# EdinburghGenomics/well_duplicates

Hardware: AMD Instinct MI355X
Metric: target x neighbour seq-compares/sec (whole node) (higher is better)
Workload: dtype u8; 1 GPU; 1 lane(s) x 96 tiles (hiseq_x) x 2500 targets x 5 levels, 50 bp; one lane per GPU (BASELINE configs[1]); lanes_per_rank=1, resident_bytes_per_rank=21098102688, mode=eq, k=0, early_exit=True, clusters_per_tile=4309253, valid_targets_per_rank=168032, parallelism=tiles sharded, 1 rank(s)

## Files before the change

### well_duplicates_amd/csrc/scan_queue.inc

```
constexpr int kFinishAllMax = 64;
#ifndef WD_QCAP
#define WD_QCAP 128
#endif
#ifndef WD_Q_OCC_IL
#define WD_Q_OCC_IL 8
#endif
constexpr int kQCap = WD_QCAP;
#ifndef WD_Q_DEPTH
#define WD_Q_DEPTH 1
#endif
constexpr int kQDepth = WD_Q_DEPTH;
constexpr int kFinishInPlace = 40;
static_assert(kQCap >= kPass && kQCap >= kFinishAllMax,
              "after a drain one pass must fit the queue, and q_finish_all adds up its pieces in the idle queue buffer");

template <typename T>
__device__ inline T late_arg(int offset)
{
    static_assert(sizeof(T) == 4 || sizeof(T) == 8, "one or two dwords");
    const __attribute__((address_space(4))) char *kp =
        (const __attribute__((address_space(4))) char *)__builtin_amdgcn_kernarg_segment_ptr();
    T v;
    if constexpr (sizeof(T) == 8)
        asm volatile("s_load_dwordx2 %0, %1, %2\n\ts_waitcnt lgkmcnt(0)" : "=s"(v) : "s"(kp), "s"(offset) : "memory");
    else
        asm volatile("s_load_dword %0, %1, %2\n\ts_waitcnt lgkmcnt(0)" : "=s"(v) : "s"(kp), "s"(offset) : "memory");
    return v;
}
#define WD_LATE_ARG(field) late_arg<decltype(ScanArgs::field)>((int)offsetof(ScanArgs, field))

struct QEnv {
    const int32_t *s_centre;
    const int32_t *s_off;
    uint32_t *s_d;
    const uint32_t *s_tid;
    gbytes base0;
    const uint8_t *const *ptab;
    int64_t stride;
    int levels, L, k, tile, t_first;
};

template <bool STRIDED, int WS = 1>
__device__ inline gbytes q_plane(const QEnv &v, int j)
{
    if (WS == 4)
        return v.base0 + (int64_t)(j >> 2) * v.stride + (j & 3);
    return STRIDED ? v.base0 + (int64_t)j * v.stride : as_global(v.ptab[j]);
}

__device__ inline void q_record_dup(const QEnv &v, int tl, int e, int dist)
{
    const int32_t *o = v.s_off + tl * (v.levels + 1);
    const int rel0 = o[0];
    int lev = 0;
    for (int l = 1; l < v.levels; l++)
        lev += (e >= o[l] - rel0) ? 1 : 0;
    atomicAdd(&v.s_d[tl * v.levels + lev], 1u);
    if (WD_LATE_ARG(log_hits)) {
        gptr<const ScanRare> rp = as_gptr(WD_LATE_ARG(rare));
        gptr<const int32_t> perm = as_gptr(WD_LATE_ARG(perm));
        wd_hit *const hits = rp->hits;
        const long long hit_cap = rp->hit_cap;
// ... 324 lines not shown
                alive = lev2_alive(st);
                if (last && alive)
                    q_record_dup(v, tl, (int)(ent.y & 0xFFFu), lev2_dist(st));
            }
            if (!last) {
                const uint64_t m = __ballot(alive);
                if (alive) {
                    const int pos = n2 + __builtin_amdgcn_mbcnt_hi((uint32_t)(m >> 32),
                                             __builtin_amdgcn_mbcnt_lo((uint32_t)m, 0u));
                    qb[pos] = make_uint2(idx, (ent.y & 0xFF000FFFu) | (st << 12));
                }
                n2 += __popcll(m);
            }
        }
        q_wave_sync();
        uint2 *t = qa; qa = qb; qb = t;
        n = last ? 0 : n2;
        j += nb;
        nb = WS == 4 ? NB : (nb < 4 ? nb * 2 : NB);
    }
    qn = 0;
}

constexpr int kLev2Closed = -1;
template <bool STRIDED, int B1, int LEVH = 0, int WS = 1>
__global__ __launch_bounds__(kBlock, LEVH > 0 ? 4 : (WS == 4 ? WD_Q_OCC_IL : 6)) void k_scan_q(ScanArgs a)
{
    static_assert(WS == 1 || (WS == 4 && STRIDED && ((B1 == 4 && LEVH == 0) || (B1 == 8 && (LEVH == 1 || LEVH == kLev2Closed)))),
                  "the interleaved layout is read a dword (4 cycles) at a time: one for equality / Hamming, "
                  "two for the first round of Levenshtein <= 2 / <= 3");
    using Entry = typename std::conditional<LEVH <= 0, uint2, uint4>::type;
    using LevS = LevState<(LEVH > 0 ? LEVH : 1)>;
    extern __shared__ uint32_t smem[];
    const int lane = threadIdx.x & (kWave - 1);
    const int wave = __builtin_amdgcn_readfirstlane(threadIdx.x >> 6);
    const int levels = a.levels;
    const int L = a.L;
    const int k = a.k;
    const int tpb = a.tpb;
    const int ncnt = 1 + 5 * levels;
    const int chunks = (a.T + tpb - 1) / tpb;
    const int nb = (int)gridDim.x, per_xcd = (nb + kXcds - 1) / kXcds;
    int vb = (int)(blockIdx.x % kXcds) * per_xcd + (int)(blockIdx.x / kXcds);
    if (nb % kXcds) {
        const int big = nb % kXcds, x = (int)(blockIdx.x % kXcds), small = nb / kXcds;
        vb = (x < big ? x * (small + 1) : big * (small + 1) + (x - big) * small) + (int)(blockIdx.x / kXcds);
    }
    const int tile = vb / chunks;
    const int chunk = vb - tile * chunks;
    const int t_first = chunk * tpb;
    const int n_t = min(tpb, a.T - t_first);

    uint32_t *s_cnt = smem;
    int32_t *s_centre = (int32_t *)(s_cnt + ncnt);
    int32_t *s_off = s_centre + tpb;
    uint32_t *s_d = (uint32_t *)(s_off + tpb * (levels + 1));
    uint32_t *s_valid = s_d + tpb * levels;
    uint32_t *s_items = s_valid + tpb;
    uint32_t *s_misc = s_items + kMaxPasses * tpb;
    const int q_base = (int)((((s_misc + 4) - smem) + 3) & ~3);
    Entry *q_a = (Entry *)(smem + q_base) + wave * 2 * kQCap;
    Entry *q_b = q_a + kQCap;

    gbytes filt = as_global(a.filter[tile]);
    const uint8_t *const *ptab = STRIDED ? nullptr : a.planes + (size_t)tile * L;
    gbytes base0 = STRIDED ? as_global(a.planes[tile]) : nullptr;
// ... 100 lines not shown
                for (int q = 0; q < NW; q++) {
                    w0[g][q] = w0[g - 1][q];
                    w1[g][q] = w1[g - 1][q];
                }
            }

            {
                it0 = s_items[wave + kWaves * min(s, n_my - 1)];
                const int tl = (int)(it0 >> 8);
                const int base = (int)(it0 & 0xFFu) * kPass;
                const int off0 = __builtin_amdgcn_readfirstlane(s_off[tl * (levels + 1)]);
                const int K = __builtin_amdgcn_readfirstlane(s_off[tl * (levels + 1) + levels]) - off0;
                const int e0 = base + lane, e1 = e0 + kWave;
                i0_0 = (uint32_t)a.nbr[off0 + min(e0, K - 1)];
                i1_0 = (uint32_t)a.nbr[off0 + min(e1, K - 1)];
            }
            if (lane == kWave - 1)
                i1_2 = (uint32_t)s_centre[it[SB] >> 8];
            if (WS == 4) {
#pragma unroll
                for (int g = 0; g < B1 / 4; g++) {
                    const int64_t go = (int64_t)min(g, max((L + 3) / 4 - 1, 0)) * stride;
                    w0_2[g] = *(const __attribute__((address_space(1))) uint32_t *)(base0 + go + (size_t)i0_2 * 4);
                    w1_2[g] = *(const __attribute__((address_space(1))) uint32_t *)(base0 + go + (size_t)i1_2 * 4);
                }
            } else if (L > 0) {
#pragma unroll
                for (int q = 0; q < B1; q++) {
                    w0_2[q] = ldb(pp[q], i0_2);
                    w1_2[q] = ldb(pp[q], i1_2);
                }
            }
            if (s >= AGE) {
                const int tl = (int)(it3 >> 8);
                const int base = (int)(it3 & 0xFFu) * kPass;
                const int off0 = __builtin_amdgcn_readfirstlane(s_off[tl * (levels + 1)]);
                const int K = __builtin_amdgcn_readfirstlane(s_off[tl * (levels + 1) + levels]) - off0;
                const int e0 = base + lane, e1 = e0 + kWave;
                const bool a0 = e0 < K, a1 = lane < kWave - 1 && e1 < K;
                if constexpr (LEVH == 0) {
                    int mm0 = 0, mm1 = 0;
                    if constexpr (WS == 4) {
                        static_assert(B1 == 4, "one dword is the first round");
                        const uint32_t cw = lev2_codes4((uint32_t)__builtin_amdgcn_readlane((int)w1_3[0], kWave - 1));
                        const uint32_t keep = L >= 4 ? (kLev2Nib & 0xFFFFu) : (((1u << (4 * L)) - 1u) & kLev2Nib);
                        const uint32_t y0 = lev2_codes4(w0_3[0]) ^ cw, y1 = lev2_codes4(w1_3[0]) ^ cw;
                        mm0 = __popc((y0 | (y0 >> 1) | (y0 >> 2)) & keep);
                        mm1 = __popc((y1 | (y1 >> 1) | (y1 >> 2)) & keep);
                    } else {
#pragma unroll
                        for (int q = 0; q < B1; q++) {
                            if (q < L) {
                                const uint32_t cc = code_of((uint32_t)__builtin_amdgcn_readlane((int)w1_3[q], kWave - 1));
                                mm0 += code_of(w0_3[q]) != cc ? 1 : 0;
                                mm1 += code_of(w1_3[q]) != cc ? 1 : 0;
                            }
                        }
                    }
                    const bool al0 = a0 && mm0 <= k, al1 = a1 && mm1 <= k;
                    const uint64_t m0 = __ballot(al0), m1 = __ballot(al1);
                    if (m0 | m1) {
                        if (B1 >= L) {
                            if (al0)
                                q_record_dup(env, tl, e0, mm0);
                            if (al1)
                                q_record_dup(env, tl, e1, mm1);
// ... 136 lines not shown
                        s1.finish(L, ch, cap, k);
                        if (a0 && s0.dup(k))
                            q_record_dup(env, tl, e0, s0.dist());
                        if (a1 && s1.dup(k))
                            q_record_dup(env, tl, e1, s1.dist());
                    } else {
                        const bool al0 = a0 && s0.alive(k, B1, ch, L, cap);
                        const bool al1 = a1 && s1.alive(k, B1, ch, L, cap);
                        const uint64_t m0 = __ballot(al0), m1 = __ballot(al1);
                        if (m0 | m1) {
                            const int n0 = __popcll(m0), n1 = __popcll(m1);
                            if (qn + n0 + n1 > kQCap)
                                q_drain_lev<STRIDED, (LEVH > 0 ? LEVH : 1), WS>(env, (uint4 *)q_a, (uint4 *)q_b, qn, B1, lane);
                            if (al0) {
                                const int pos = qn + __builtin_amdgcn_mbcnt_hi((uint32_t)(m0 >> 32),
                                                         __builtin_amdgcn_mbcnt_lo((uint32_t)m0, 0u));
                                const uint64_t pk = lev_pack(s0, ch);
                                ((uint4 *)q_a)[pos] = make_uint4(i0_3, ((uint32_t)tl << 24) | (uint32_t)e0,
                                                                 (uint32_t)pk, (uint32_t)(pk >> 32));
                            }
                            if (al1) {
                                const int pos = qn + n0 + __builtin_amdgcn_mbcnt_hi((uint32_t)(m1 >> 32),
                                                              __builtin_amdgcn_mbcnt_lo((uint32_t)m1, 0u));
                                const uint64_t pk = lev_pack(s1, ch);
                                ((uint4 *)q_a)[pos] = make_uint4(i1_3, ((uint32_t)tl << 24) | (uint32_t)e1,
                                                                 (uint32_t)pk, (uint32_t)(pk >> 32));
                            }
                            qn += n0 + n1;
                        }
                    }
                }
            }
        }
        if (qn > 0) {
            if constexpr (LEVH == 0)
                q_drain<STRIDED, 8, WS>(env, (uint2 *)q_a, (uint2 *)q_b, qn, B1, lane);
            else if constexpr (LEVH == kLev2Closed)
                q_drain_lev2<STRIDED, WS>(env, (uint2 *)q_a, (uint2 *)q_b, qn, B1, lane);
            else
                q_drain_lev<STRIDED, LEVH, WS>(env, (uint4 *)q_a, (uint4 *)q_b, qn, B1, lane);
        }
    }
    __syncthreads();

    uint32_t acc_wells = 0, acc_dups = 0, acc_hit = 0, acc_first = 0, acc_last = 0, acc_valid = 0;
    gptr<uint32_t> const out_pt = as_gptr(WD_LATE_ARG(out_per_target));
    gptr<const int32_t> const perm = out_pt ? as_gptr(WD_LATE_ARG(perm)) : nullptr;
    const size_t T_all = (size_t)WD_LATE_ARG(T);
    for (int tl = wave; tl < n_t; tl += kWaves) {
        const bool valid = __builtin_amdgcn_readfirstlane(s_valid[tl]) != 0;
        gptr<uint32_t> opt = out_pt ? out_pt + ((size_t)tile * T_all + (perm ? perm[t_first + tl] : t_first + tl)) * levels
                                    : nullptr;
        if (!valid) {
            if (opt && lane < levels)
                opt[lane] = WD_INVALID_TARGET;
            continue;
        }
        uint32_t my_d = 0, my_w = 0;
        if (lane < levels) {
            my_d = s_d[tl * levels + lane];
            my_w = (uint32_t)(s_off[tl * (levels + 1) + lane + 1] - s_off[tl * (levels + 1) + lane]);
        }
        const uint64_t hm = __ballot(lane < levels && my_d > 0);
        acc_valid += 1;
        acc_wells += my_w;
        acc_dups += my_d;
        acc_hit += my_d ? 1u : 0u;
        if (hm) {
            acc_first += (lane == __ffsll((long long)hm) - 1) ? 1u : 0u;
            acc_last += (lane == 63 - __clzll((long long)hm)) ? 1u : 0u;
        }
        if (opt && lane < levels)
            opt[lane] = my_d;
    }
    if (lane < levels) {
        if (acc_wells) atomicAdd(&s_cnt[1 + lane], acc_wells);
        if (acc_dups) atomicAdd(&s_cnt[1 + levels + lane], acc_dups);
        if (acc_hit) atomicAdd(&s_cnt[1 + 2 * levels + lane], acc_hit);
        if (acc_first) atomicAdd(&s_cnt[1 + 3 * levels + lane], acc_first);
        if (acc_last) atomicAdd(&s_cnt[1 + 4 * levels + lane], acc_last);
    }
    if (lane == 0 && acc_valid)
        atomicAdd(&s_cnt[0], acc_valid);
    __syncthreads();
    unsigned long long *const out_tile = WD_LATE_ARG(out_tile);
    for (int i = threadIdx.x; i < ncnt; i += kBlock) {
        const uint32_t v = s_cnt[i];
        if (v)
            g_atomic_add(&out_tile[(size_t)tile * ncnt + i], (unsigned long long)v);
    }
}
```

### well_duplicates_amd/csrc/wd_ctx.h

```cpp
#ifndef WD_CTX_H
#define WD_CTX_H
#include "wd_shared.h"

constexpr int kLaneTopMaxPasses = 8;

struct wd_ctx {
    int device = 0;
    hipStream_t own_stream = nullptr;
    hipStream_t stream = nullptr;
    std::string err;

    int early_exit = 1;
    int tpb = 64;
    int batch_first = 4;
    int batch_next = 4;
    int queue_kernel = 1;
    int queue_first = 0;
    int dense_kernel = -1;
    int dense_tile_chunk = 16;
    uint32_t *d_sig = nullptr;
    size_t sig_cap = 0;
    unsigned long long *d_partial = nullptr;
    size_t partial_cap = 0;
    uint32_t *d_mask = nullptr;
// ... 28 lines not shown
    int64_t P = 0;
    int32_t *d_centre = nullptr, *d_lvl_off = nullptr, *d_nbr = nullptr;
    int64_t idx_min = 0, idx_max = -1;
    int64_t k_max = 0;
    std::vector<long long> h_gbase;
    void *d_nbr_t = nullptr;
    bool nbr_t16 = false;
    int32_t *d_rel_t = nullptr;
    void *d_udelta = nullptr;
    uint8_t *d_guni = nullptr;
    int32_t *d_ginfo = nullptr;
    uint16_t *d_uoff = nullptr;
    int2 *d_useg = nullptr;
    int32_t *d_wdelta = nullptr;
    uint8_t *d_wlev = nullptr;
    uint32_t *d_wmask = nullptr;
    uint8_t *d_wfull = nullptr;
    int dense_sym = 1;
    bool dense_sym_on = false;
    int32_t centre0 = 0;
    int win_kpad = 0;
    int win_dwords = 0;
    long long n_uniform_groups = -1, n_window_groups = -1;
    int32_t *d_pblocks = nullptr;
    int n_pblocks = 0;
    uint32_t *d_tblflags = nullptr;
    long long *d_gbase = nullptr;
    bool has_targets = false;
    bool has_empty_level = false;

    std::vector<const uint8_t *> h_tbl;
    const uint8_t **d_tbl = nullptr;
    size_t d_tbl_cap = 0;
    uint32_t *d_status = nullptr;
    uint32_t *h_status = nullptr;
    ScanRare *d_rare = nullptr;
    ScanRare h_rare = {nullptr, nullptr, nullptr, 0};

    unsigned long long *d_out_tile = nullptr;
    size_t d_out_tile_cap = 0;
    uint32_t *d_out_pt = nullptr;
    size_t d_out_pt_cap = 0;
    uint8_t *d_stage = nullptr;
    size_t d_stage_cap = 0;

    wd_hit *d_hits = nullptr;
    unsigned long long *d_hit_count = nullptr;
    int64_t hit_cap = 0;
    uint8_t *d_gather = nullptr;
    size_t gather_cap = 0;
    size_t hit_alloc = 0;

    std::vector<std::pair<hipEvent_t, hipEvent_t>> events;
    std::vector<std::pair<hipEvent_t, hipEvent_t>> free_events;
    double prof_ms = 0.0;
    int64_t prof_launches = 0;

    void *comm = nullptr;

    struct IngestSlot {
        uint8_t *pinned = nullptr;
        size_t cap = 0;
        uint8_t *dev = nullptr;
        size_t dev_cap = 0;
        uint8_t *file = nullptr;
        size_t file_cap = 0;
// ... 135 lines not shown
```

### well_duplicates_amd/csrc/wd_shared.h

```cpp
#ifndef WD_SHARED_H
#define WD_SHARED_H
#include <hip/hip_runtime.h>

#include <dlfcn.h>
#include <zlib.h>
#include <stdint.h>
#include <stdio.h>
#include <stdlib.h>
#include <string.h>

#include <fcntl.h>
#include <emmintrin.h>
#include <sched.h>
#include <sys/stat.h>
#include <unistd.h>

#include <algorithm>
#include <atomic>
#include <chrono>
#include <condition_variable>
#include <functional>
#include <new>
#include <system_error>
#include <memory>
// ... 6 lines not shown

#include "welldup.h"

constexpr int kWave = 64;
constexpr int kBlock = 256;
constexpr int kWaves = kBlock / kWave;
constexpr int kMaxLevels = WD_MAX_LEVELS;
constexpr int kCounters = 1 + 5 * kMaxLevels;
constexpr uint32_t kStatusEmptyLevel = 1u;
constexpr int kXcds = 8;
constexpr int kMaxTpb = 64;
constexpr int kPass = 127;
constexpr int kMaxPasses = 4;

constexpr int lev_first(int H) { return H == 1 ? 7 : H == 2 ? 10 : H == 3 ? 13 : H == 4 ? 16 : H <= 6 ? 20 : 24; }

constexpr int kDenseChainVersion = 5;
constexpr int kSigCycles = 10;
constexpr int kRowGroups = 4;
constexpr int kDenseMaxK = 1 << 17;

struct ScanArgs {
    const uint8_t *const *planes;
    const uint8_t *const *filter;
    int64_t stride;
    const int32_t *centre;
    const int32_t *lvl_off;
    const int32_t *nbr;
    unsigned long long *out_tile;
    uint32_t *out_per_target;
    const struct ScanRare *rare;
    const int32_t *perm;
    int T, levels, L, k, tpb, early, check_empty, log_hits;
};

struct ScanRare {
    uint32_t *status;
    wd_hit *hits;
    unsigned long long *hit_count;
    long long hit_cap;
};

struct InfJob;
struct InfResult;

#endif
```

### well_duplicates_amd/csrc/welldup_core.hip

```cpp
#include "wd_ctx.h"

namespace {

#include "synth_kernels.inc"

struct Id128 { char b[WD_UNIQUE_ID_BYTES]; };
struct Rccl {
    void *handle = nullptr;
    int (*GetUniqueId)(void *) = nullptr;
    int (*CommInitRank)(void **, int, Id128, int) = nullptr;
    int (*AllReduce)(const void *, void *, size_t, int, int, void *, hipStream_t) = nullptr;
    int (*CommDestroy)(void *) = nullptr;
    const char *(*GetErrorString)(int) = nullptr;
};
Rccl g_rccl;

bool rccl_load(std::string &err)
{
    if (g_rccl.handle)
        return true;
    const char *names[] = {"librccl.so.1", "librccl.so", "/opt/rocm/lib/librccl.so.1"};
    void *h = nullptr;
    for (const char *n : names) {
        h = dlopen(n, RTLD_NOW | RTLD_GLOBAL);
// ... 148 lines not shown
void wd_destroy(wd_ctx *ctx)
{
    if (!ctx)
        return;
    (void)hipSetDevice(ctx->device);
    (void)hipStreamSynchronize(ctx->stream);
    if (ctx->fast_exit) {
        (void)hipDeviceSynchronize();
        if (ctx->comm && g_rccl.CommDestroy)
            g_rccl.CommDestroy(ctx->comm);
        delete ctx;
        return;
    }
    const bool lap_on = getenv("WD_INFLATE_STATS") != nullptr;
    auto lap_t = std::chrono::steady_clock::now();
    auto lap = [&](const char *what) {
        if (!lap_on)
            return;
        const auto now = std::chrono::steady_clock::now();
        fprintf(stderr, "[wd close] %-28s %6.1f ms\n", what, 1e3 * std::chrono::duration<double>(now - lap_t).count());
        lap_t = now;
    };
    drain_events(ctx);
    for (auto &ev : ctx->free_events) {
        (void)hipEventDestroy(ev.first);
        (void)hipEventDestroy(ev.second);
    }
    if (ctx->comm && g_rccl.CommDestroy)
        g_rccl.CommDestroy(ctx->comm);
    (void)hipFree(ctx->d_centre);
    (void)hipFree(ctx->d_lvl_off);
    (void)hipFree(ctx->d_nbr);
    (void)hipFree(ctx->d_tbl);
    (void)hipFree(ctx->d_status);
    (void)hipFree(ctx->d_rare);
    (void)hipFree(ctx->d_nbr_t);
    (void)hipFree(ctx->d_rel_t);
    (void)hipFree(ctx->d_udelta);
    (void)hipFree(ctx->d_guni);
    (void)hipFree(ctx->d_ginfo);
    (void)hipFree(ctx->d_uoff);
    (void)hipFree(ctx->d_useg);
    (void)hipFree(ctx->d_wdelta);
    (void)hipFree(ctx->d_wlev);
    (void)hipFree(ctx->d_wmask);
    (void)hipFree(ctx->d_wfull);
    (void)hipFree(ctx->d_tblflags);
    (void)hipFree(ctx->d_mark);
    (void)hipFree(ctx->d_sig);
    (void)hipFree(ctx->d_partial);
    (void)hipFree(ctx->d_mask);
    (void)hipFree(ctx->d_queue);
    (void)hipFree(ctx->d_qcnt);
    (void)hipFree(ctx->d_cand);
    (void)hipFree(ctx->d_pblocks);
    (void)hipFree(ctx->d_centre_q);
    (void)hipFree(ctx->d_lvl_off_q);
    (void)hipFree(ctx->d_perm);
    drop_line_tables(ctx);
    for (hipStream_t q : {ctx->dense_hi, ctx->dense_lo})
        if (q) {
            (void)hipStreamSynchronize(q);
            (void)hipStreamDestroy(q);
        }
    for (hipEvent_t e : {ctx->dense_ev_start, ctx->dense_ev_done, ctx->dense_ev_cmp[0], ctx->dense_ev_cmp[1],
                         ctx->dense_ev_pack[0], ctx->dense_ev_pack[1]})
// ... 108 lines not shown
        if (value != 1 && value != 4)
            return WD_ERR_ARG;
        ctx->well_stride = (int)value;
    } else if (n == "fast_inflate") {
        ctx->fast_inflate = value ? 1 : 0;
    } else if (n == "dense_overlap") {
        ctx->dense_overlap = value ? 1 : 0;
    } else if (n == "dense_pack_blocks") {
        if (value < 0 || value > (1 << 24))
            return WD_ERR_ARG;
        ctx->dense_pack_blocks = (int)value;
    } else if (n == "dense_part_tiles") {
        if (value < 0 || value > 65535)
            return WD_ERR_ARG;
        ctx->dense_part_tiles = (int)value;
    } else if (n == "line_walk") {
        ctx->line_walk = value < 0 ? -1 : (value ? 1 : 0);
    } else if (n == "line_pairs") {
        if (value < 0 || value > (1 << 20))
            return WD_ERR_ARG;
        if (value != ctx->line_pairs) {
            WD_HIP(ctx, hipStreamSynchronize(ctx->stream));
            drop_line_tables(ctx);
        }
        ctx->line_pairs = (int)value;
    } else if (n == "sort_targets") {
        ctx->sort_targets = value ? 1 : 0;
    } else if (n == "sort_strip") {
        if (value < 0 || value > (1 << 20))
            return WD_ERR_ARG;
        ctx->sort_strip = (int)value;
    } else if (n == "lev2_closed") {
        ctx->lev2_closed = value ? 1 : 0;
    } else if (n == "test_thread_limit") {
        ctx->test_thread_limit = value;
    } else if (n == "inflate_waves") {
        if (value != 0 && value != 1 && value != 4 && value != 8)
            return WD_ERR_ARG;
        ctx->inflate_waves = (int)value;
    } else if (n == "inflate_chunk_mb") {
        if (value < 1 || value > 1024)
            return WD_ERR_ARG;
        ctx->inflate_chunk_bytes = (size_t)value << 20;
    } else if (n == "inflate_warm") {
        if (value) {
            WD_HIP(ctx, hipSetDevice(ctx->device));
            return inflate_prepare_shared(ctx, wd_ctx::kInflateChunks);
        }
    } else if (n == "dense_pack") {
        ctx->dense_pack = value < 0 ? -1 : (value ? 1 : 0);
    } else if (n == "dense_windows") {
        ctx->dense_windows = value ? 1 : 0;
    } else if (n == "dense_sym") {
        if (ctx->dense_sym != (value ? 1 : 0)) {
            WD_HIP(ctx, hipStreamSynchronize(ctx->stream));
            drop_dense_tables(ctx);
        }
        ctx->dense_sym = value ? 1 : 0;
    } else if (n == "dense_nt") {
        ctx->dense_nt = value ? 1 : 0;
    } else if (n == "dense_queue_cap") {
        if (value < 0)
            return WD_ERR_ARG;
        ctx->dense_queue_cap = value;
    } else if (n == "queue_kernel") {
        ctx->queue_kernel = value ? 1 : 0;
// ... 3 lines not shown
        ctx->queue_first = (int)value;
    } else {
        return fail(ctx, WD_ERR_ARG, "unknown option " + n);
    }
    return WD_OK;
} WD_CATCH

int wd_get_option(wd_ctx *ctx, const char *name, int64_t *value)
try {
    if (!ctx || !name || !value)
        return WD_ERR_ARG;
    std::string n(name);
    if (n == "early_exit") *value = ctx->early_exit;
    else if (n == "targets_per_block") *value = ctx->tpb;
    else if (n == "batch_first") *value = ctx->batch_first;
    else if (n == "batch_next") *value = ctx->batch_next;
    else if (n == "profile") *value = ctx->profile;
    else if (n == "queue_kernel") *value = ctx->queue_kernel;
    else if (n == "fast_exit") *value = ctx->fast_exit;
    else if (n == "hitlog_capacity") *value = ctx->hit_cap;
    else if (n == "dense_kernel") *value = ctx->dense_kernel;
    else if (n == "dense_tile_chunk") *value = ctx->dense_tile_chunk;
    else if (n == "dense_queue_cap") *value = ctx->dense_queue_cap;
    else if (n == "dense_pack") *value = ctx->dense_pack;
    else if (n == "dense_windows") *value = ctx->dense_windows;
    else if (n == "dense_sym") *value = ctx->dense_sym;
    else if (n == "dense_sym_on") *value = ctx->dense_sym_on ? 1 : 0;
    else if (n == "dense_nt") *value = ctx->dense_nt;
    else if (n == "fast_inflate") *value = ctx->fast_inflate;
    else if (n == "inflate_chunk_mb") *value = (long long)(ctx->inflate_chunk_bytes >> 20);
    else if (n == "inflate_waves") *value = ctx->inflate_waves;
    else if (n == "test_thread_limit") *value = ctx->test_thread_limit;
    else if (n == "lev2_closed") *value = ctx->lev2_closed;
    else if (n == "sort_targets") *value = ctx->sort_targets;
    else if (n == "line_walk") *value = ctx->line_walk;
    else if (n == "line_pairs") *value = ctx->line_pairs;
    else if (n == "line_walk_blocks") *value = ctx->lw_blocks;
    else if (n == "sort_strip") *value = ctx->sort_strip;
    else if (n == "dense_overlap") *value = ctx->dense_overlap;
    else if (n == "dense_part_tiles") *value = ctx->dense_part_tiles;
    else if (n == "dense_pack_blocks") *value = ctx->dense_pack_blocks;
    else if (n == "inflate_files_gpu") *value = ctx->inflate_files_gpu.load();
    else if (n == "inflate_files_host") *value = ctx->inflate_files_host.load();
    else if (n == "inflate_files_early") *value = ctx->inflate_files_early.load();
    else if (n == "inflate_us_per_file") *value = ctx->inflate_us_per_file.load();
    else if (n == "well_stride") *value = ctx->well_stride;
    else if (n == "null_stream") *value = ctx->stream == nullptr ? 1 : 0;
    else if (n == "queue_first") *value = ctx->queue_first;
    else if (n == "dense_uniform_groups") *value = ctx->n_uniform_groups;
    else if (n == "dense_window_groups") *value = ctx->n_window_groups < 0 || ctx->dense_windows ? ctx->n_window_groups : 0;
    else if (n == "dense_window_dwords") *value = ctx->win_dwords;
    else if (n == "lane_top_passes") *value = ctx->lane_top_passes;
    else if (n == "lane_top_max_passes") *value = kLaneTopMaxPasses;
    else return fail(ctx, WD_ERR_ARG, "unknown option " + n);
    return WD_OK;
} WD_CATCH

int wd_malloc(wd_ctx *ctx, size_t bytes, void **out_dev)
try {
    if (!ctx || !out_dev)
        return WD_ERR_ARG;
    if (bind_device(ctx))
        return WD_ERR_HIP;
    *out_dev = nullptr;
    WD_HIP(ctx, hipMalloc(out_dev, bytes ? bytes : 1));
    return WD_OK;
// ... 273 lines not shown
```

### well_duplicates_amd/csrc/welldup_queue.hip

```cpp
#include "wd_ctx.h"

#ifndef WD_UNIT_ID
#define WD_UNIT_ID "unknown"
#endif
namespace wd { const char *unit_id_queue() { return WD_UNIT_ID; } }

using namespace wd;

namespace {

#include "device_common.inc"
#include "scan_sequential.inc"
#include "lev2_stream.inc"
#include "scan_queue.inc"

#define WD_LAUNCH_Q(STR, B1_, LEVH_, WS_, LDS_)                                                          \
    do {                                                                                                 \
        snprintf(ctx->last_kernel, sizeof(ctx->last_kernel), "k_scan_q<%s, %d, %d, %d>%s", (STR) ? "true" : "false", \
                 (int)(B1_), (int)(LEVH_), (int)(WS_), a.perm ? ", targets sorted by centre" : "");      \
        hipLaunchKernelGGL((k_scan_q<(STR), (B1_), (LEVH_), (WS_)>), grid, dim3(kBlock), (LDS_), ctx->stream, a); \
    } while (0)


template <bool STRIDED>
int launch_queue_t(wd_ctx *ctx, const ScanArgs &a, dim3 grid)
{
    const size_t lds = (size_t)scan_q_lds_dwords(a.levels, a.tpb) * sizeof(uint32_t);
    if (STRIDED && ctx->well_stride == 4) {
        WD_LAUNCH_Q(true, 4, 0, STRIDED ? 4 : 1, lds);
        return 0;
    }
    int first = ctx->queue_first;
    if (first == 0)
        first = a.k <= 0 ? 2 : (a.k == 1 ? 3 : (a.k == 2 ? 5 : (a.k == 3 ? 6 : 8)));
    switch (first) {
    case 1: WD_LAUNCH_Q(STRIDED, 1, 0, 1, lds); break;
    case 2: WD_LAUNCH_Q(STRIDED, 2, 0, 1, lds); break;
    case 3: WD_LAUNCH_Q(STRIDED, 3, 0, 1, lds); break;
    case 4: WD_LAUNCH_Q(STRIDED, 4, 0, 1, lds); break;
    case 5: WD_LAUNCH_Q(STRIDED, 5, 0, 1, lds); break;
    case 6: WD_LAUNCH_Q(STRIDED, 6, 0, 1, lds); break;
    case 7: WD_LAUNCH_Q(STRIDED, 7, 0, 1, lds); break;
    default: WD_LAUNCH_Q(STRIDED, 8, 0, 1, lds); break;
    }
    return 0;
}

template <bool STRIDED, int H>
void launch_queue_lev_t(wd_ctx *ctx, const ScanArgs &a, dim3 grid)
{
    if constexpr (H == 1) {
        if (a.k == 2 && ctx->lev2_closed) {
            const size_t lds2 = (size_t)scan_q_lds_dwords(a.levels, a.tpb, 2) * sizeof(uint32_t);
// ... 13 lines not shown
    }
    const size_t lds = (size_t)scan_q_lds_dwords(a.levels, a.tpb, 4) * sizeof(uint32_t);
    if constexpr (STRIDED && H == 1) {
        if (ctx->well_stride == 4) {
            WD_LAUNCH_Q(true, 8, 1, 4, lds);
            return;
        }
    }
    constexpr int first_even = lev_first(H) - (H <= 2 ? 2 : 0), first_odd = lev_first(H) + 1 - (H == 1 ? 2 : 0);
    if (a.k & 1)
        WD_LAUNCH_Q(STRIDED, first_odd, H, 1, lds);
    else
        WD_LAUNCH_Q(STRIDED, first_even, H, 1, lds);
}


}

namespace wd {

int launch_queue(wd_ctx *ctx, const ScanArgs &a, dim3 grid, bool strided)
{
    return strided ? launch_queue_t<true>(ctx, a, grid) : launch_queue_t<false>(ctx, a, grid);
}

void launch_queue_lev(wd_ctx *ctx, const ScanArgs &a, dim3 grid, bool strided, int h)
{
    if (h <= 1) { if (strided) launch_queue_lev_t<true, 1>(ctx, a, grid); else launch_queue_lev_t<false, 1>(ctx, a, grid); }
    else if (h == 2) { if (strided) launch_queue_lev_t<true, 2>(ctx, a, grid); else launch_queue_lev_t<false, 2>(ctx, a, grid); }
    else { if (strided) launch_queue_lev_t<true, 3>(ctx, a, grid); else launch_queue_lev_t<false, 3>(ctx, a, grid); }
}

}
```

### well_duplicates_amd/csrc/welldup_scan.hip

```cpp
#include "wd_ctx.h"

#ifndef WD_UNIT_ID
#define WD_UNIT_ID "unknown"
#endif
namespace wd { const char *unit_id_scan() { return WD_UNIT_ID; } }

using namespace wd;

namespace {

#include "device_common.inc"
#include "scan_sequential.inc"
#include "scan_lev_generic.inc"
#include "gen_rings.inc"

constexpr int kHamShapes[][2] = {{2, 4}, {3, 4}, {4, 4}, {4, 8}, {8, 8}};
constexpr int kLevB2 = 8;

template <bool STRIDED>
void launch_ham(wd_ctx *ctx, const ScanArgs &a, dim3 grid)
{
    const int b1 = ctx->batch_first, b2 = ctx->batch_next;
#define WD_CASE(B1, B2)                                                                   \
    if (b1 == B1 && b2 == B2) {                                                           \
        snprintf(ctx->last_kernel, sizeof(ctx->last_kernel), "k_scan<HamState, %s, %d, %d>", STRIDED ? "true" : "false", B1, B2); \
        hipLaunchKernelGGL((k_scan<HamState, STRIDED, B1, B2>), grid, dim3(kBlock), 0,    \
                           ctx->stream, a);                                               \
        return;                                                                           \
    }
    WD_CASE(2, 4)
    WD_CASE(3, 4)
    WD_CASE(4, 4)
    WD_CASE(4, 8)
    WD_CASE(8, 8)
#undef WD_CASE
}

template <int H>
void launch_lev(wd_ctx *ctx, const ScanArgs &a, dim3 grid, bool strided)
{
    snprintf(ctx->last_kernel, sizeof(ctx->last_kernel), "k_scan<LevState<%d>, %s, %d, %d>", H, strided ? "true" : "false",
             lev_first(H), kLevB2);
    if (strided)
        hipLaunchKernelGGL((k_scan<LevState<H>, true, lev_first(H), kLevB2>), grid, dim3(kBlock), 0,
                           ctx->stream, a);
    else
        hipLaunchKernelGGL((k_scan<LevState<H>, false, lev_first(H), kLevB2>), grid, dim3(kBlock), 0,
// ... 142 lines not shown
    ctx->k_max = 0;
    for (int t = 0; t < T; t++)
        ctx->k_max = std::max<int64_t>(ctx->k_max, (int64_t)lvl_off[(size_t)t * row + levels] - lvl_off[(size_t)t * row]);
    set_group_bases(ctx, lvl_off, T, levels);
    if (int rc = install_sorted_view(ctx, centre, lvl_off, T, levels, row_length_of(centre, lvl_off, nbr, T, levels)))
        return rc;
    ctx->has_targets = true;
    return WD_OK;
} WD_CATCH

int wd_scan_async(wd_ctx *ctx, int n_tiles, int L, int mode, int k, const uint8_t *const *planes,
                  const uint8_t *const *filter, int64_t N, int64_t *out_tile_dev,
                  uint32_t *out_per_target_dev)
try {
    if (!ctx)
        return WD_ERR_ARG;
    if (!ctx->has_targets)
        return fail(ctx, WD_ERR_STATE, "wd_set_targets has not been called");
    if (n_tiles < 0 || L < 0 || N < 0 || !out_tile_dev)
        return fail(ctx, WD_ERR_ARG, "bad n_tiles, L, N or out_tile");
    if (mode != WD_MODE_EQ && mode != WD_MODE_HAMMING && mode != WD_MODE_LEVENSHTEIN)
        return fail(ctx, WD_ERR_ARG, "bad mode");
    if (n_tiles > 0 && (!filter || (L > 0 && !planes)))
        return fail(ctx, WD_ERR_ARG, "null plane/filter table");
    if (!valid_batches(ctx->batch_first, ctx->batch_next))
        return fail(ctx, WD_ERR_ARG, "unsupported batch_first/batch_next pair");
    if (bind_device(ctx))
        return WD_ERR_HIP;
    if (ctx->T > 0 && n_tiles > 0 && (ctx->idx_min < 0 || ctx->idx_max >= N))
        return fail(ctx, WD_ERR_INDEX, "a target index lies outside [0, N)");

    const int levels = ctx->levels;
    const size_t ncnt = 1 + 5 * (size_t)levels;
    WD_HIP(ctx, hipMemsetAsync(out_tile_dev, 0, (size_t)n_tiles * ncnt * sizeof(int64_t), ctx->stream));
    if (n_tiles == 0 || ctx->T == 0)
        return WD_OK;

    int kk = k;
    bool lev = false;
    if (mode == WD_MODE_EQ) {
        kk = 0;
    } else if (mode == WD_MODE_LEVENSHTEIN) {
        if (k >= L) {
            kk = L;
            lev = ctx->hit_cap > 0 && L >= 2 && lev_generic_lds_bytes(L, L / 2) <= 64 * 1024;
        } else if (k >= 2) {
            lev = true;
        }
    }
    if (kk > L)
        kk = L;
    if (kk < -1)
        kk = -1;
    const bool lev_generic = lev && kk / 2 > 8;
    if (lev_generic && lev_generic_lds_bytes(L, kk / 2) > 64 * 1024)
        return fail(ctx, WD_ERR_UNSUPPORTED,
                    "Levenshtein threshold k >= 18 with this read length needs more than 64 KB of LDS");

    bool strided = L > 0;
    int64_t stride = 0;
    const int ws = ctx->well_stride;
    if (ws == 4) {
        if (L > 4)
            stride = (int64_t)(planes[4] - planes[0]);
        for (int i = 0; i < n_tiles; i++) {
            const uint8_t *b = planes[(size_t)i * L];
            if (L > 0 && ((uintptr_t)b & 3u))
                return fail(ctx, WD_ERR_ARG, "interleaved planes must start 4-byte aligned");
            for (int c = 0; c < L; c++)
// ... 72 lines not shown
        const int part = dense_part_size(ctx, n_tiles, tile_chunk);
        if (!dense_rows_reserve(ctx, part * (part < n_tiles ? 2 : 1), N))
            use_dense = false;
    }
    if (ws == 4 && ctx->dense_kernel < 0)
        use_dense = false;
    const int chunks = (ctx->T + ctx->tpb - 1) / ctx->tpb;
    const long long dense_bpt = (ctx->T + kBlock - 1) / kBlock;
    const long long dense_blocks = (long long)kXcds * ((dense_bpt + kXcds - 1) / kXcds) *
                                   ((n_tiles + tile_chunk - 1) / tile_chunk);
    const long long nblocks = lev_generic ? (long long)ctx->T * n_tiles
                              : use_dense ? dense_blocks
                                          : (long long)chunks * n_tiles;
    if (nblocks > 0x7FFFFFFFll)
        return fail(ctx, WD_ERR_UNSUPPORTED, "grid too large; raise targets_per_block");
    dim3 grid((unsigned)nblocks);

    const bool use_queue = !lev && ctx->queue_kernel && ctx->early_exit && kk <= 254 &&
                           ctx->k_max <= (int64_t)kMaxPasses * kPass;
    const bool lev_queue_il = lev && !lev_generic && kk / 2 == 1 && ctx->queue_kernel && ctx->early_exit &&
                              ctx->k_max <= (int64_t)kMaxPasses * kPass;

    bool use_lines = false;
    if (line_walk_wanted(ctx) && !use_dense && (ws == 1 || strided) && ctx->queue_kernel && ctx->early_exit && L >= 1 && levels <= 8 &&
        ((!lev && kk <= 254) || (lev && kk == 2 && ctx->lev2_closed && !lev_generic))) {
        if (int rc = build_line_tables(ctx))
            return rc;
        use_lines = ctx->lw_blocks > 0;
    }
    if (ws == 4 && (use_dense || !strided || !(use_lines || use_queue || lev_queue_il)))
        return fail(ctx, WD_ERR_UNSUPPORTED,
                    "the interleaved layout is read by the queue kernel and the line walk only (equality, Hamming, "
                    "Levenshtein <= 3)");

    std::pair<hipEvent_t, hipEvent_t> ev{nullptr, nullptr};
    const bool timed = ctx->profile > 0 && (ctx->profile_seq++ % ctx->profile) == 0;
    if (timed) {
        if (!ctx->free_events.empty()) {
            ev = ctx->free_events.back();
            ctx->free_events.pop_back();
        } else {
            WD_HIP(ctx, hipEventCreate(&ev.first));
            WD_HIP(ctx, hipEventCreate(&ev.second));
        }
        WD_HIP(ctx, hipEventRecord(ev.first, ctx->stream));
    }
    if (use_dense) {
        int rc = launch_dense(ctx, a, n_tiles, N, strided, n_plane_ptrs, tile_chunk, lev2);
        if (rc)
            return rc;
        snprintf(ctx->last_kernel, sizeof(ctx->last_kernel), "dense chain v%d, %s%s (k_dense_sig .. k_dense_reduce)",
                 kDenseChainVersion, lev2 ? "Levenshtein <= 2" : (kk > 0 ? "Hamming" : "equality"),
                 ctx->dense_sym_on ? ", pairs from one end" : "");
    } else if (use_lines) {
        const int first = kk <= 0 ? 2 : (kk == 1 ? 3 : (kk == 2 ? 5 : (kk == 3 ? 6 : 8)));
        const int rc = launch_lines(ctx, a, n_tiles, lev, first, strided);
        if (rc)
            return rc;
    } else if (use_queue) {
        queue_view(ctx, a);
        launch_queue(ctx, a, grid, strided);
    } else if (!lev) {
        if (strided)
            launch_ham<true>(ctx, a, grid);
        else
            launch_ham<false>(ctx, a, grid);
    } else if (lev && !lev_generic && kk / 2 <= 3 && ctx->queue_kernel && ctx->early_exit &&
               ctx->k_max <= (int64_t)kMaxPasses * kPass) {
        const int h = kk / 2;
        queue_view(ctx, a);
        launch_queue_lev(ctx, a, grid, strided, h);
    } else if (lev_generic) {
        const int h = kk / 2;
        const size_t lds = lev_generic_lds_bytes(L, h);
        snprintf(ctx->last_kernel, sizeof(ctx->last_kernel), "k_scan_lev_generic<%s>", strided ? "true" : "false");
        if (strided)
            hipLaunchKernelGGL((k_scan_lev_generic<true>), grid, dim3(kWave), lds, ctx->stream, a, h);
        else
            hipLaunchKernelGGL((k_scan_lev_generic<false>), grid, dim3(kWave), lds, ctx->stream, a, h);
    } else {
        const int h = kk / 2;
        if (h <= 1) launch_lev<1>(ctx, a, grid, strided);
        else if (h <= 2) launch_lev<2>(ctx, a, grid, strided);
        else if (h <= 3) launch_lev<3>(ctx, a, grid, strided);
        else if (h <= 4) launch_lev<4>(ctx, a, grid, strided);
        else if (h <= 6) launch_lev<6>(ctx, a, grid, strided);
        else launch_lev<8>(ctx, a, grid, strided);
    }
    WD_HIP(ctx, hipGetLastError());
    if (timed) {
        WD_HIP(ctx, hipEventRecord(ev.second, ctx->stream));
        ctx->events.push_back(ev);
    }
    return WD_OK;
} WD_CATCH

int wd_scan_status(wd_ctx *ctx)
{
    if (!ctx)
        return WD_ERR_ARG;
    if (bind_device(ctx))
        return WD_ERR_HIP;
    WD_HIP(ctx, hipMemcpyAsync(ctx->h_status, ctx->d_status, sizeof(uint32_t), hipMemcpyDeviceToHost, ctx->stream));
    WD_HIP(ctx, hipMemsetAsync(ctx->d_status, 0, sizeof(uint32_t), ctx->stream));
    WD_HIP(ctx, hipStreamSynchronize(ctx->stream));
    if (*ctx->h_status & kStatusEmptyLevel)
        return fail(ctx, WD_ERR_EMPTY_LEVEL, "a target with a valid centre has an empty level");
    return WD_OK;
}

int wd_count_tiles(wd_ctx *ctx, int n_tiles, int L, int mode, int k, const uint8_t *const *planes,
                   const uint8_t *const *filter, int64_t N, int64_t *out_tile,
                   uint32_t *out_per_target)
try {
    if (!ctx || !out_tile)
        return WD_ERR_ARG;
    if (!ctx->has_targets)
        return fail(ctx, WD_ERR_STATE, "wd_set_targets has not been called");
    if (n_tiles < 0)
        return fail(ctx, WD_ERR_ARG, "bad n_tiles");
    if (bind_device(ctx))
        return WD_ERR_HIP;
    const size_t ncnt = 1 + 5 * (size_t)ctx->levels;
    const size_t n_out = std::max<size_t>(1, (size_t)n_tiles * ncnt);
    const size_t n_pt = std::max<size_t>(1, (size_t)n_tiles * ctx->T * ctx->levels);
    int rc = grow(ctx, ctx->d_out_tile, ctx->d_out_tile_cap, n_out);
    if (rc)
        return rc;
    if (out_per_target) {
        rc = grow(ctx, ctx->d_out_pt, ctx->d_out_pt_cap, n_pt);
        if (rc)
            return rc;
    }
    std::vector<const uint8_t *> dev_planes, dev_filter;
    if (n_tiles > 0 && planes && filter && L >= 0 && N >= 0) {
        auto on_device = [](const void *p) {
            hipPointerAttribute_t at;
            if (hipPointerGetAttributes(&at, p) != hipSuccess) {
// ... 224 lines not shown
```

Baseline: 115.7 billion compares/s.

## Replace per-call output memset with self-resetting chunk-counting accumulators; add optional launch stagger

```diff
diff --git a/well_duplicates_amd/csrc/scan_queue.inc b/well_duplicates_amd/csrc/scan_queue.inc
--- a/well_duplicates_amd/csrc/scan_queue.inc
+++ b/well_duplicates_amd/csrc/scan_queue.inc
@@ -28,6 +28,45 @@
     return v;
 }
 #define WD_LATE_ARG(field) late_arg<decltype(ScanArgs::field)>((int)offsetof(ScanArgs, field))
+
+#include "tally_accum.inc"
+
+constexpr int kStaggerSleep = 16;
+constexpr int kStaggerMaxNaps = 4096;
+__device__ inline void q_stagger(int ticks, int resident)
+{
+    const uint32_t r = blockIdx.x / kXcds;
+    if ((int)r >= resident)
+        return;
+    uint32_t h = (r + 1u) * 0x9E3779B1u;
+    h ^= h >> 15;
+    h *= 0x85EBCA77u;
+    h ^= h >> 13;
+    if ((h & 3u) == 0)
+        return;
+    const uint64_t delay = 1u + (h >> 2) % (uint32_t)ticks;
+    const uint64_t t0 = wall_clock64();
+    for (int nap = 0; nap < kStaggerMaxNaps && wall_clock64() - t0 < delay; nap++)
+        __builtin_amdgcn_s_sleep(kStaggerSleep);
+}
+
+#ifdef WD_Q_STAMPS
+constexpr int kQStampBlocks = 1 << 16;
+__device__ unsigned long long g_q_stamps[4 * kQStampBlocks];
+#define WD_Q_STAMP(slot)                                                      \
+    do {                                                                      \
+        if (threadIdx.x == 0 && blockIdx.x < (unsigned)kQStampBlocks)         \
+            g_q_stamps[4 * blockIdx.x + (slot)] = wall_clock64();             \
+    } while (0)
+#define WD_Q_STAMP_CLEAR(slot)                                                \
+    do {                                                                      \
+        if (threadIdx.x == 0 && blockIdx.x < (unsigned)kQStampBlocks)         \
+            g_q_stamps[4 * blockIdx.x + (slot)] = 0ull;                       \
+    } while (0)
+#else
+#define WD_Q_STAMP(slot) do { } while (0)
+#define WD_Q_STAMP_CLEAR(slot) do { } while (0)
+#endif
 
 struct QEnv {
     const int32_t *s_centre;
@@ -418,6 +457,11 @@
     using Entry = typename std::conditional<LEVH <= 0, uint2, uint4>::type;
     using LevS = LevState<(LEVH > 0 ? LEVH : 1)>;
     extern __shared__ uint32_t smem[];
+    WD_Q_STAMP(0);
+    WD_Q_STAMP_CLEAR(1);
+    WD_Q_STAMP_CLEAR(2);
+    if (a.stagger_ticks > 0)
+        q_stagger(a.stagger_ticks, a.resident_wgs);
     const int lane = threadIdx.x & (kWave - 1);
     const int wave = __builtin_amdgcn_readfirstlane(threadIdx.x >> 6);
     const int levels = a.levels;
@@ -584,6 +628,10 @@
                 }
             }
             if (s >= AGE) {
+#ifdef WD_Q_STAMPS
+                if (s == AGE)
+                    WD_Q_STAMP(1);
+#endif
                 const int tl = (int)(it3 >> 8);
                 const int base = (int)(it3 & 0xFFu) * kPass;
                 const int off0 = __builtin_amdgcn_readfirstlane(s_off[tl * (levels + 1)]);
@@ -786,6 +834,7 @@
                 }
             }
         }
+        WD_Q_STAMP(2);
         if (qn > 0) {
             if constexpr (LEVH == 0)
                 q_drain<STRIDED, 8, WS>(env, (uint2 *)q_a, (uint2 *)q_b, qn, B1, lane);
@@ -838,9 +887,19 @@
         atomicAdd(&s_cnt[0], acc_valid);
     __syncthreads();
     unsigned long long *const out_tile = WD_LATE_ARG(out_tile);
-    for (int i = threadIdx.x; i < ncnt; i += kBlock) {
-        const uint32_t v = s_cnt[i];
-        if (v)
-            g_atomic_add(&out_tile[(size_t)tile * ncnt + i], (unsigned long long)v);
-    }
-}
+    unsigned long long *const acc = WD_LATE_ARG(acc);
+    if (acc) {
+        const int tpb_l = WD_LATE_ARG(tpb);
+        const int n_chunks = ((int)T_all + tpb_l - 1) / tpb_l;
+        for (int i = threadIdx.x; i < ncnt; i += kBlock)
+            tally_arrive(as_gptr(acc + (size_t)tile * ncnt + i), as_gptr(out_tile + (size_t)tile * ncnt + i),
+                         (unsigned long long)s_cnt[i], n_chunks);
+    } else {
+        for (int i = threadIdx.x; i < ncnt; i += kBlock) {
+            const uint32_t v = s_cnt[i];
+            if (v)
+                g_atomic_add(&out_tile[(size_t)tile * ncnt + i], (unsigned long long)v);
+        }
+    }
+    WD_Q_STAMP(3);
+}
diff --git a/well_duplicates_amd/csrc/tally_accum.inc b/well_duplicates_amd/csrc/tally_accum.inc
--- /dev/null
+++ b/well_duplicates_amd/csrc/tally_accum.inc
@@ -0,0 +1,38 @@
+#ifndef TALLY_ATOMIC_ADD
+#define TALLY_ATOMIC_ADD(p, v) __hip_atomic_fetch_add((p), (v), __ATOMIC_RELAXED, __HIP_MEMORY_SCOPE_AGENT)
+#endif
+
+constexpr int kTallyCountShift = 48;
+constexpr unsigned long long kTallyValueMask = (1ull << kTallyCountShift) - 1;
+constexpr long long kTallyMaxChunks = 65534;
+
+__host__ __device__ inline unsigned long long tally_pack(unsigned long long value)
+{
+    return (value & kTallyValueMask) | (1ull << kTallyCountShift);
+}
+
+__host__ __device__ inline bool tally_complete(unsigned long long old, int chunks)
+{
+    return (long long)(old >> kTallyCountShift) == (long long)chunks - 1;
+}
+
+__host__ __device__ inline unsigned long long tally_total(unsigned long long old, unsigned long long mine)
+{
+    return (old + mine) & kTallyValueMask;
+}
+
+template <class AccPtr, class OutPtr>
+__host__ __device__ inline void tally_arrive(AccPtr acc, OutPtr out, unsigned long long value, int chunks)
+{
+    const unsigned long long mine = tally_pack(value);
+#ifdef WD_ACC_SPLIT_ADD
+    const unsigned long long old = TALLY_ATOMIC_ADD(acc, 1ull << kTallyCountShift);
+    TALLY_ATOMIC_ADD(acc, mine & kTallyValueMask);
+#else
+    const unsigned long long old = TALLY_ATOMIC_ADD(acc, mine);
+#endif
+    if (tally_complete(old, chunks)) {
+        *out = tally_total(old, mine);
+        TALLY_ATOMIC_ADD(acc, 0ull - (old + mine));
+    }
+}
diff --git a/well_duplicates_amd/csrc/wd_ctx.h b/well_duplicates_amd/csrc/wd_ctx.h
--- a/well_duplicates_amd/csrc/wd_ctx.h
+++ b/well_duplicates_amd/csrc/wd_ctx.h
@@ -84,6 +84,12 @@
     std::vector<const uint8_t *> h_tbl;
     const uint8_t **d_tbl = nullptr;
     size_t d_tbl_cap = 0;
+    unsigned long long *d_acc = nullptr;
+    size_t d_acc_cap = 0;
+    bool acc_dirty = false;
+    int scan_accum = 1;
+    int scan_stagger = 0;
+    int wall_khz = 0;
     uint32_t *d_status = nullptr;
     uint32_t *h_status = nullptr;
     ScanRare *d_rare = nullptr;
diff --git a/well_duplicates_amd/csrc/wd_shared.h b/well_duplicates_amd/csrc/wd_shared.h
--- a/well_duplicates_amd/csrc/wd_shared.h
+++ b/well_duplicates_amd/csrc/wd_shared.h
@@ -62,6 +62,9 @@
     const struct ScanRare *rare;
     const int32_t *perm;
     int T, levels, L, k, tpb, early, check_empty, log_hits;
+    unsigned long long *acc;
+    int stagger_ticks;
+    int resident_wgs;
 };
 
 struct ScanRare {
diff --git a/well_duplicates_amd/csrc/welldup_core.hip b/well_duplicates_amd/csrc/welldup_core.hip
--- a/well_duplicates_amd/csrc/welldup_core.hip
+++ b/well_duplicates_amd/csrc/welldup_core.hip
@@ -204,6 +204,7 @@
     (void)hipFree(ctx->d_lvl_off);
     (void)hipFree(ctx->d_nbr);
     (void)hipFree(ctx->d_tbl);
+    (void)hipFree(ctx->d_acc);
     (void)hipFree(ctx->d_status);
     (void)hipFree(ctx->d_rare);
     (void)hipFree(ctx->d_nbr_t);
@@ -378,6 +379,12 @@
         ctx->sort_strip = (int)value;
     } else if (n == "lev2_closed") {
         ctx->lev2_closed = value ? 1 : 0;
+    } else if (n == "scan_accum") {
+        ctx->scan_accum = value ? 1 : 0;
+    } else if (n == "scan_stagger") {
+        if (value < 0 || value > 1000)
+            return WD_ERR_ARG;
+        ctx->scan_stagger = (int)value;
     } else if (n == "test_thread_limit") {
         ctx->test_thread_limit = value;
     } else if (n == "inflate_waves") {
@@ -447,6 +454,8 @@
     else if (n == "inflate_waves") *value = ctx->inflate_waves;
     else if (n == "test_thread_limit") *value = ctx->test_thread_limit;
     else if (n == "lev2_closed") *value = ctx->lev2_closed;
+    else if (n == "scan_accum") *value = ctx->scan_accum;
+    else if (n == "scan_stagger") *value = ctx->scan_stagger;
     else if (n == "sort_targets") *value = ctx->sort_targets;
     else if (n == "line_walk") *value = ctx->line_walk;
     else if (n == "line_pairs") *value = ctx->line_pairs;
diff --git a/well_duplicates_amd/csrc/welldup_queue.hip b/well_duplicates_amd/csrc/welldup_queue.hip
--- a/well_duplicates_amd/csrc/welldup_queue.hip
+++ b/well_duplicates_amd/csrc/welldup_queue.hip
@@ -14,11 +14,35 @@
 #include "lev2_stream.inc"
 #include "scan_queue.inc"
 
+template <auto KERNEL>
+int resident_per_xcd(const wd_ctx *ctx, size_t lds)
+{
+    struct Shape { int device; size_t lds; int wgs; };
+    static std::mutex mu;
+    static std::vector<Shape> known;
+    std::lock_guard<std::mutex> lock(mu);
+    for (const Shape &s : known)
+        if (s.device == ctx->device && s.lds == lds)
+            return s.wgs;
+    int per_cu = 0, cus = 0;
+    if (hipOccupancyMaxActiveBlocksPerMultiprocessor(&per_cu, KERNEL, kBlock, lds) != hipSuccess ||
+        hipDeviceGetAttribute(&cus, hipDeviceAttributeMultiprocessorCount, ctx->device) != hipSuccess) {
+        (void)hipGetLastError();
+        per_cu = 0;
+    }
+    const int wgs = std::max(0, per_cu) * std::max(1, cus / kXcds);
+    known.push_back(Shape{ctx->device, lds, wgs});
+    return wgs;
+}
+
 #define WD_LAUNCH_Q(STR, B1_, LEVH_, WS_, LDS_)                                                          \
     do {                                                                                                 \
         snprintf(ctx->last_kernel, sizeof(ctx->last_kernel), "k_scan_q<%s, %d, %d, %d>%s", (STR) ? "true" : "false", \
                  (int)(B1_), (int)(LEVH_), (int)(WS_), a.perm ? ", targets sorted by centre" : "");      \
-        hipLaunchKernelGGL((k_scan_q<(STR), (B1_), (LEVH_), (WS_)>), grid, dim3(kBlock), (LDS_), ctx->stream, a); \
+        ScanArgs qa_ = a;                                                                                \
+        if (qa_.stagger_ticks > 0)                                                                       \
+            qa_.resident_wgs = resident_per_xcd<k_scan_q<(STR), (B1_), (LEVH_), (WS_)>>(ctx, (LDS_));    \
+        hipLaunchKernelGGL((k_scan_q<(STR), (B1_), (LEVH_), (WS_)>), grid, dim3(kBlock), (LDS_), ctx->stream, qa_); \
     } while (0)
 
 
@@ -98,3 +122,16 @@
 }
 
 }
+
+#ifdef WD_Q_STAMPS
+extern "C" int wd_q_stamps(wd_ctx *ctx, unsigned long long *out, int n_blocks)
+{
+    if (!ctx || !out || n_blocks < 0 || n_blocks > kQStampBlocks)
+        return WD_ERR_ARG;
+    if (bind_device(ctx))
+        return WD_ERR_HIP;
+    WD_HIP(ctx, hipStreamSynchronize(ctx->stream));
+    WD_HIP(ctx, hipMemcpyFromSymbol(out, HIP_SYMBOL(g_q_stamps), (size_t)n_blocks * 4 * sizeof(unsigned long long)));
+    return WD_OK;
+}
+#endif
diff --git a/well_duplicates_amd/csrc/welldup_scan.hip b/well_duplicates_amd/csrc/welldup_scan.hip
--- a/well_duplicates_amd/csrc/welldup_scan.hip
+++ b/well_duplicates_amd/csrc/welldup_scan.hip
@@ -13,6 +13,19 @@
 #include "scan_sequential.inc"
 #include "scan_lev_generic.inc"
 #include "gen_rings.inc"
+#include "tally_accum.inc"
+
+int reserve_accumulators(wd_ctx *ctx, size_t n)
+{
+    const size_t had = ctx->d_acc_cap;
+    if (int rc = grow(ctx, ctx->d_acc, ctx->d_acc_cap, n))
+        return rc;
+    if (ctx->d_acc_cap != had || ctx->acc_dirty) {
+        WD_HIP(ctx, hipMemsetAsync(ctx->d_acc, 0, ctx->d_acc_cap * sizeof(unsigned long long), ctx->stream));
+        ctx->acc_dirty = false;
+    }
+    return WD_OK;
+}
 
 constexpr int kHamShapes[][2] = {{2, 4}, {3, 4}, {4, 4}, {4, 8}, {8, 8}};
 constexpr int kLevB2 = 8;
@@ -221,9 +234,10 @@
 
     const int levels = ctx->levels;
     const size_t ncnt = 1 + 5 * (size_t)levels;
-    WD_HIP(ctx, hipMemsetAsync(out_tile_dev, 0, (size_t)n_tiles * ncnt * sizeof(int64_t), ctx->stream));
-    if (n_tiles == 0 || ctx->T == 0)
+    if (n_tiles == 0 || ctx->T == 0) {
+        WD_HIP(ctx, hipMemsetAsync(out_tile_dev, 0, (size_t)n_tiles * ncnt * sizeof(int64_t), ctx->stream));
         return WD_OK;
+    }
 
     int kk = k;
     bool lev = false;
@@ -362,6 +376,30 @@
         return fail(ctx, WD_ERR_UNSUPPORTED,
                     "the interleaved layout is read by the queue kernel and the line walk only (equality, Hamming, "
                     "Levenshtein <= 3)");
+
+    const bool lev_queue = lev && !lev_generic && kk / 2 <= 3 && ctx->queue_kernel && ctx->early_exit &&
+                           ctx->k_max <= (int64_t)kMaxPasses * kPass;
+    const bool runs_scan_q = !use_dense && !use_lines && (use_queue || lev_queue);
+    const bool use_acc = runs_scan_q && ctx->scan_accum && chunks <= kTallyMaxChunks;
+    a.acc = nullptr;
+    a.stagger_ticks = 0;
+    a.resident_wgs = 0;
+    if (use_acc) {
+        if (int rc = reserve_accumulators(ctx, (size_t)n_tiles * ncnt))
+            return rc;
+        a.acc = ctx->d_acc;
+    } else {
+        WD_HIP(ctx, hipMemsetAsync(out_tile_dev, 0, (size_t)n_tiles * ncnt * sizeof(int64_t), ctx->stream));
+    }
+    if (runs_scan_q && ctx->scan_stagger > 0) {
+        if (ctx->wall_khz == 0) {
+            int khz = 0;
+            if (hipDeviceGetAttribute(&khz, hipDeviceAttributeWallClockRate, ctx->device) != hipSuccess || khz <= 0)
+                khz = 100000;
+            ctx->wall_khz = khz;
+        }
+        a.stagger_ticks = (int)std::max<long long>(1, (long long)ctx->scan_stagger * ctx->wall_khz / 1000);
+    }
 
     std::pair<hipEvent_t, hipEvent_t> ev{nullptr, nullptr};
     const bool timed = ctx->profile > 0 && (ctx->profile_seq++ % ctx->profile) == 0;
@@ -395,8 +433,7 @@
             launch_ham<true>(ctx, a, grid);
         else
             launch_ham<false>(ctx, a, grid);
-    } else if (lev && !lev_generic && kk / 2 <= 3 && ctx->queue_kernel && ctx->early_exit &&
-               ctx->k_max <= (int64_t)kMaxPasses * kPass) {
+    } else if (lev_queue) {
         const int h = kk / 2;
         queue_view(ctx, a);
         launch_queue_lev(ctx, a, grid, strided, h);
@@ -417,7 +454,10 @@
         else if (h <= 6) launch_lev<6>(ctx, a, grid, strided);
         else launch_lev<8>(ctx, a, grid, strided);
     }
-    WD_HIP(ctx, hipGetLastError());
+    if (const hipError_t e = hipGetLastError(); e != hipSuccess) {
+        ctx->acc_dirty = ctx->acc_dirty || use_acc;
+        return fail(ctx, WD_ERR_HIP, std::string("scan launch: ") + hipGetErrorString(e));
+    }
     if (timed) {
         WD_HIP(ctx, hipEventRecord(ev.second, ctx->stream));
         ctx->events.push_back(ev);
@@ -433,7 +473,10 @@
         return WD_ERR_HIP;
     WD_HIP(ctx, hipMemcpyAsync(ctx->h_status, ctx->d_status, sizeof(uint32_t), hipMemcpyDeviceToHost, ctx->stream));
     WD_HIP(ctx, hipMemsetAsync(ctx->d_status, 0, sizeof(uint32_t), ctx->stream));
-    WD_HIP(ctx, hipStreamSynchronize(ctx->stream));
+    if (const hipError_t e = hipStreamSynchronize(ctx->stream); e != hipSuccess) {
+        ctx->acc_dirty = true;
+        return fail(ctx, WD_ERR_HIP, std::string("hipStreamSynchronize(ctx->stream): ") + hipGetErrorString(e));
+    }
     if (*ctx->h_status & kStatusEmptyLevel)
         return fail(ctx, WD_ERR_EMPTY_LEVEL, "a target with a valid centre has an empty level");
     return WD_OK;
```

Result: no change. 115.7 billion compares/s, median of 2 (-0.0%).
